# mit-han-lab/qserve

Measured on NVIDIA H100. Metric: tokens/s Llama-3-8B W4A8KV4 decode b64, higher is better.
Workload: dtype s8

## Files before the change

### qserve_b200/csrc/gemm.cu

```cuda
#include <cstdarg>
#include <cstdio>
#include <cstdlib>
#include <cstring>
#include <mutex>
#include <unordered_map>

#include "common.cuh"
#include "launch.h"

namespace qs {

namespace {

constexpr int kBM = 128;
constexpr int kBK = 128;
constexpr int kSub = 2;
constexpr int kConsumers = 128;
constexpr int kNumThreads = 192;
constexpr int kFrag = 4;

enum { kModeW4Chn = 0, kModeW4Grp = 1, kModeW8 = 2 };

struct GemmParams {
  const uint8_t* s2_scales;
  const uint8_t* s2_zeros;
  const __half* wscales;
  const __half* w_szs;
  const __half* ascales;
  const __half* a_ssums;
  __half* out;
  int32_t* acc_out;
  int M, N, K;
  int m_tiles, kb_per_tile, split;
  unsigned long long* prof;
};

template <int MODE, int NT, int WS, int AS>
struct Cfg {
  static constexpr int kActSub = NT * kBK;
  static constexpr int kWSub = (MODE == kModeW8) ? kBM * kBK : kBM * kBK / 2;
  static constexpr int kS2Sub = (MODE == kModeW4Grp) ? 2 * kBM : 0;
  static constexpr int kActBytes = kSub * kActSub;
  static constexpr int kWBytes = kSub * kWSub;
  static constexpr int kS2Bytes = kSub * kS2Sub;
  static constexpr int kWStageTx = kWBytes + kS2Bytes;
  static constexpr int kOffAct = 0;
  static constexpr int kOffW = kOffAct + AS * kActBytes;
  static constexpr int kOffS2 = kOffW + WS * kWBytes;
  static constexpr int kPipeBytes = kOffS2 + WS * kS2Bytes;
  static constexpr int kRedBytes = NT * kBM * 4;
  static constexpr int kOffRow = (kPipeBytes > kRedBytes ? kPipeBytes : kRedBytes);
  static constexpr int kOffBar = kOffRow + 2 * NT * 4;
  static constexpr int kNumBars = 2 * WS + 2 * AS;
  static constexpr int kSmemBytes = kOffBar + kNumBars * 8;
  static constexpr int kCtasPerSm = (NT <= 64 && kSmemBytes <= 113 * 1024) ? 2 : 1;
  static_assert(kSmemBytes <= 227 * 1024, "shared memory overflow");
};

__device__ __forceinline__ unsigned long long gtime() {
  unsigned long long t;
  asm volatile("mov.u64 %0, %globaltimer;" : "=l"(t)::"memory");
  return t;
}
#define QS_PROF(slot) do { if (p.prof) p.prof[blockIdx.x * 16 + (slot)] = gtime(); } while (0)

__device__ __forceinline__ uint32_t cluster_ctarank() {
  uint32_t r;
  asm volatile("mov.u32 %0, %%cluster_ctarank;" : "=r"(r));
  return r;
}
__device__ __forceinline__ void cluster_sync_all() {
  asm volatile("barrier.cluster.arrive.release.aligned;\n\tbarrier.cluster.wait.acquire.aligned;" ::: "memory");
}
__device__ __forceinline__ void cluster_arrive() { asm volatile("barrier.cluster.arrive.release;" ::: "memory"); }
__device__ __forceinline__ void cluster_wait() { asm volatile("barrier.cluster.wait.acquire;" ::: "memory"); }
__device__ __forceinline__ uint32_t smid() {
  uint32_t r;
  asm volatile("mov.u32 %0, %%smid;" : "=r"(r));
  return r;
}
__device__ __forceinline__ uint32_t map_to_cta(uint32_t smem_addr, uint32_t rank) {
  uint32_t r;
  asm volatile("mapa.shared::cluster.u32 %0, %1, %2;" : "=r"(r) : "r"(smem_addr), "r"(rank));
  return r;
}
__device__ __forceinline__ void st_dsmem_u32(uint32_t addr, uint32_t v) {
  asm volatile("st.shared::cluster.u32 [%0], %1;" ::"r"(addr), "r"(v) : "memory");
}

template <int V>
struct IntTag { static constexpr int value = V; };

template <int MODE>
__device__ __forceinline__ float epilogue_one(int32_t acc, float ws, float wsz, float as, float asum) {
  float ps = __int2float_rn(acc);
  if constexpr (MODE == kModeW4Chn) {
    float t = __fmul_rn(__fmul_rn(ps, ws), as);
    float u = __fmul_rn(wsz, asum);
    return __fsub_rn(t, u);
  } else {
    return __fmul_rn(ps, __fmul_rn(ws, as));
  }
}

template <int MODE>
__device__ __forceinline__ int acc_channel(int h, int w, int r) {
  return (MODE == kModeW8) ? 64 * h + 16 * w + r : 32 * w + 16 * h + r;
}

template <int MODE, int NT, int WS, int AS, bool ACC>
__global__ void __launch_bounds__(kNumThreads, Cfg<MODE, NT, WS, AS>::kCtasPerSm)
gemm_kernel(const __grid_constant__ CUtensorMap tmap_act, const __grid_constant__ CUtensorMap tmap_w, const GemmParams p) {
  using C = Cfg<MODE, NT, WS, AS>;
  extern __shared__ __align__(1024) uint8_t smem[];
  if (threadIdx.x == 0 && (smem_u32(smem) & 1023u) != 0) __trap();
  uint8_t* s_act = smem + C::kOffAct;
  uint8_t* s_w = smem + C::kOffW;
  uint8_t* s_s2 = smem + C::kOffS2;
  int32_t* s_red = reinterpret_cast<int32_t*>(smem);
  float* s_asc = reinterpret_cast<float*>(smem + C::kOffRow);
  float* s_asum = s_asc + NT;
  uint64_t* bar_wfull = reinterpret_cast<uint64_t*>(smem + C::kOffBar);
  uint64_t* bar_wempty = bar_wfull + WS;
  uint64_t* bar_xfull = bar_wempty + WS;
  uint64_t* bar_xempty = bar_xfull + AS;

  const int warp = threadIdx.x >> 5;
  const int lane = threadIdx.x & 31;
  const int S = p.split;
  const int rank = (S > 1) ? static_cast<int>(cluster_ctarank()) : 0;
  const int tile = blockIdx.x / S;
  const int m_tile = tile % p.m_tiles, n_tile = tile / p.m_tiles;
  const int KB = p.kb_per_tile;
  const int kb_begin = (KB * rank) / S, kb_end = (KB * (rank + 1)) / S;
  const int n_kb = kb_end - kb_begin;
  if (threadIdx.x == 0) {
    QS_PROF(0);
    if (p.prof) p.prof[blockIdx.x * 16 + 15] = smid();
  }
  qs_trace(QS_K_GEMM, 0);

  if (threadIdx.x == 0) {
    tma_prefetch_desc(&tmap_act);
    tma_prefetch_desc(&tmap_w);
    for (int i = 0; i < WS; ++i) {
      mbar_init(&bar_wfull[i], 1);
      mbar_init(&bar_wempty[i], 4);
    }
    for (int i = 0; i < AS; ++i) {
      mbar_init(&bar_xfull[i], 1);
      mbar_init(&bar_xempty[i], 4);
    }
    fence_barrier_init();
  }
  __syncthreads();
  if (threadIdx.x == 0) { pdl_launch_dependents(); QS_PROF(1); }

  if (warp == 4) {
    if (lane == 0) {
      const int w_row = (MODE == kModeW8) ? n_tile * kBM : n_tile * 4;
      const uint8_t* s2s = p.s2_scales + static_cast<size_t>(n_tile) * kBM;
      const uint8_t* s2z = p.s2_zeros + static_cast<size_t>(n_tile) * kBM;
      int s = 0;
      uint32_t ph = 0;
      for (int it = 0; it < n_kb; ++it) {
        if (it >= WS) mbar_wait_nocall(&bar_wempty[s], ph);
        mbar_expect_tx(&bar_wfull[s], C::kWStageTx);
#pragma unroll
        for (int u = 0; u < kSub; ++u) {
          const int kb = (kb_begin + it) * kSub + u;
          tma_load_2d(s_w + s * C::kWBytes + u * C::kWSub, &tmap_w, (MODE == kModeW8) ? kb * kBK : kb * 256, w_row, &bar_wfull[s]);
          if constexpr (MODE == kModeW4Grp) {
            const int kg = kb < p.K / kBK ? kb : p.K / kBK - 1;
            bulk_copy_g2s(s_s2 + s * C::kS2Bytes + u * C::kS2Sub, s2s + static_cast<size_t>(kg) * p.N, kBM, &bar_wfull[s]);
            bulk_copy_g2s(s_s2 + s * C::kS2Bytes + u * C::kS2Sub + kBM, s2z + static_cast<size_t>(kg) * p.N, kBM, &bar_wfull[s]);
          }
        }
        if (++s == WS) { s = 0; if (it >= WS) ph ^= 1; }
      }
      QS_PROF(3);
    }
  } else if (warp == 5) {
    if (lane == 0) {
      const int a_row = m_tile * NT;
      pdl_wait();
      QS_PROF(2);
      qs_trace(QS_K_GEMM, 1, 5 * 32);
      int s = 0;
      uint32_t ph = 0;
      for (int it = 0; it < n_kb; ++it) {
        if (it >= AS) mbar_wait_nocall(&bar_xempty[s], ph);
        mbar_expect_tx(&bar_xfull[s], C::kActBytes);
#pragma unroll
        for (int u = 0; u < kSub; ++u)
          tma_load_2d(s_act + s * C::kActBytes + u * C::kActSub, &tmap_act, ((kb_begin + it) * kSub + u) * kBK, a_row, &bar_xfull[s]);
        if (++s == AS) { s = 0; if (it >= AS) ph ^= 1; }
      }
    }
  } else {
    int32_t acc[2][NT / 2];
#pragma unroll
    for (int h = 0; h < 2; ++h)
#pragma unroll
      for (int i = 0; i < NT / 2; ++i) acc[h][i] = 0;
    mbar_wait_nocall(&bar_wfull[0], 0);
    mbar_wait_nocall(&bar_xfull[0], 0);
    if (threadIdx.x == 0) QS_PROF(4);
    const bool leader = lane == 0;
    int sw = 0, sx = 0, prev_sw = WS - 1, prev_sx = AS - 1;
    uint32_t phw = 0, phx = 0;
    for (int it = 0; it < n_kb; ++it) {
      mbar_wait_nocall(&bar_wfull[sw], phw);
      mbar_wait_nocall(&bar_xfull[sx], phx);
      if constexpr (MODE == kModeW8) {
#pragma unroll
        for (int u = 0; u < kSub; ++u) {
          const uint64_t bdesc = gmma_desc_sw128(smem_u32(s_act + sx * C::kActBytes + u * C::kActSub));
          const uint64_t adesc = gmma_desc_sw128(smem_u32(s_w + sw * C::kWBytes + u * C::kWSub));
          wgmma_fence();
#pragma unroll
          for (int t = 0; t < kBK / 32; ++t) {
            wgmma_s8_ss(acc[0], adesc + t * 2, bdesc + t * 2);
            wgmma_s8_ss(acc[1], adesc + (64 * kBK >> 4) + t * 2, bdesc + t * 2);
          }
          wgmma_commit();
        }
        wgmma_wait<kSub>();
        mbar_arrive_if(&bar_wempty[prev_sw], it > 0 && leader);
        mbar_arrive_if(&bar_xempty[prev_sx], it > 0 && leader);
      } else {
        uint32_t fr[kFrag][2][4];
#pragma unroll
        for (int u = 0; u < kSub; ++u) {
          const uint64_t bdesc = gmma_desc_sw128(smem_u32(s_act + sx * C::kActBytes + u * C::kActSub));
          const uint8_t* wsrc = s_w + sw * C::kWBytes + u * C::kWSub + warp * 2048 + lane * 16;
          uint32_t sc4 = 0, zp4 = 0;
          if constexpr (MODE == kModeW4Grp) {
            const uint8_t* s2 = s_s2 + sw * C::kS2Bytes + u * C::kS2Sub + warp * 32 + (lane >> 2) * 4;
            sc4 = *reinterpret_cast<const uint32_t*>(s2);
            zp4 = *reinterpret_cast<const uint32_t*>(s2 + kBM);
          }
#pragma unroll
          for (int t = 0; t < 4; ++t) {
            const int j = u * 4 + t;
            const uint4 v = *reinterpret_cast<const uint4*>(wsrc + t * 512);
            uint32_t xl = v.x & 0x0F0F0F0Fu, xh = (v.x >> 4) & 0x0F0F0F0Fu;
            uint32_t yl = v.y & 0x0F0F0F0Fu, yh = (v.y >> 4) & 0x0F0F0F0Fu;
            uint32_t zl = v.z & 0x0F0F0F0Fu, zh = (v.z >> 4) & 0x0F0F0F0Fu;
            uint32_t wl = v.w & 0x0F0F0F0Fu, wh = (v.w >> 4) & 0x0F0F0F0Fu;
            if constexpr (MODE == kModeW4Grp) {
              const uint32_t s0 = sc4 & 0xFF, s1 = (sc4 >> 8) & 0xFF, s2 = (sc4 >> 16) & 0xFF, s3 = sc4 >> 24;
              const uint32_t z0 = __byte_perm(zp4, 0, 0x0000), z1 = __byte_perm(zp4, 0, 0x1111);
              const uint32_t z2 = __byte_perm(zp4, 0, 0x2222), z3 = __byte_perm(zp4, 0, 0x3333);
              xl = __vadd4(xl * s0, z0); zl = __vadd4(zl * s0, z0);
              yl = __vadd4(yl * s1, z1); wl = __vadd4(wl * s1, z1);
              xh = __vadd4(xh * s2, z2); zh = __vadd4(zh * s2, z2);
              yh = __vadd4(yh * s3, z3); wh = __vadd4(wh * s3, z3);
            }
            wgmma_wait<kFrag - 1>();
            if (j == kFrag - 1) mbar_arrive_if(&bar_xempty[prev_sx], it > 0 && leader);
            uint32_t(&f)[2][4] = fr[j % kFrag];
            f[0][0] = xl; f[0][1] = yl; f[0][2] = zl; f[0][3] = wl;
            f[1][0] = xh; f[1][1] = yh; f[1][2] = zh; f[1][3] = wh;
            wgmma_fence();
            wgmma_s8_rs(acc[0], f[0], bdesc + t * 2);
            wgmma_s8_rs(acc[1], f[1], bdesc + t * 2);
            wgmma_commit();
          }
        }
        mbar_arrive_if(&bar_wempty[sw], leader);
      }
      prev_sw = sw;
      prev_sx = sx;
      if (++sw == WS) { sw = 0; phw ^= 1; }
      if (++sx == AS) { sx = 0; phx ^= 1; }
    }
    wgmma_wait<0>();
    if (threadIdx.x == 0) QS_PROF(6);
    if (S > 1) cluster_arrive();

    const int epi_tid = threadIdx.x;
    pdl_wait();
    const int m0 = m_tile * NT;
    for (int j = epi_tid; j < NT; j += kConsumers) {
      const bool ok = (m0 + j) < p.M;
      s_asc[j] = ok ? __half2float(p.ascales[m0 + j]) : 0.f;
      if constexpr (MODE == kModeW4Chn) s_asum[j] = ok ? __half2float(p.a_ssums[m0 + j]) : 0.f;
    }
    if (S > 1) cluster_wait(); else named_bar_sync(1, kConsumers);
    if (epi_tid == 0) QS_PROF(8);
    const int r0 = lane >> 2, c0 = (lane & 3) * 2;
    if (S == 1) {
#pragma unroll
      for (int h = 0; h < 2; ++h)
#pragma unroll
        for (int i = 0; i < NT / 2; ++i) {
          const int ch = acc_channel<MODE>(h, warp, r0 + 8 * ((i >> 1) & 1));
          const int tok = (i >> 2) * 8 + c0 + (i & 1);
          s_red[tok * kBM + ch] = acc[h][i];
        }
    } else {
      const int cps = kBM / S;
      const uint32_t rx_base = smem_u32(s_red);
#pragma unroll
      for (int h = 0; h < 2; ++h)
#pragma unroll
        for (int i = 0; i < NT / 2; ++i) {
          const int ch = acc_channel<MODE>(h, warp, r0 + 8 * ((i >> 1) & 1));
          const int tok = (i >> 2) * 8 + c0 + (i & 1);
          const uint32_t owner = static_cast<uint32_t>(ch / cps);
          st_dsmem_u32(map_to_cta(rx_base, owner) + static_cast<uint32_t>(((rank * NT + tok) * cps + ch % cps) * 4), static_cast<uint32_t>(acc[h][i]));
        }
    }
    if (epi_tid == 0) QS_PROF(9);
  }
  if (S > 1 && threadIdx.x >= kConsumers) { cluster_arrive(); cluster_wait(); }

  if (S > 1) cluster_sync_all(); else __syncthreads();
  if (threadIdx.x < kConsumers) {
    pdl_wait();
    const int tid = threadIdx.x;
    if (tid == 0) QS_PROF(10);
    const int npairs = 64 / S;
    const int pr = (64 * rank) / S + tid % npairs;
    const float ws0 = __half2float(__ldg(p.wscales + n_tile * kBM + 2 * pr)), ws1 = __half2float(__ldg(p.wscales + n_tile * kBM + 2 * pr + 1));
    float wz0 = 0.f, wz1 = 0.f;
    if constexpr (MODE == kModeW4Chn) {
      wz0 = __half2float(__ldg(p.w_szs + n_tile * kBM + 2 * pr));
      wz1 = __half2float(__ldg(p.w_szs + n_tile * kBM + 2 * pr + 1));
    }
    const int m0 = m_tile * NT;
    const int tstep = kConsumers / npairs;
    const int n = n_tile * kBM + 2 * pr;
    const int tok_end = min(NT, p.M - m0);
    const int tok0 = tid / npairs;
    const uint32_t off0 = static_cast<uint32_t>((tok0 * kBM + 2 * pr) * 4), off_step = static_cast<uint32_t>(tstep * kBM * 4);
    __half* optr = p.out + static_cast<size_t>(m0 + tok0) * p.N + n;
    const size_t ostep = static_cast<size_t>(tstep) * p.N;
    auto finish = [&](int tok, int2 acc, __half* dst) {
      const float as = s_asc[tok], asum = s_asum[tok];
      const float o0 = epilogue_one<MODE>(acc.x, ws0, wz0, as, asum);
      const float o1 = epilogue_one<MODE>(acc.y, ws1, wz1, as, asum);
      *reinterpret_cast<__half2*>(dst) = __floats2half2_rn(o0, o1);
      if constexpr (ACC) *reinterpret_cast<int2*>(p.acc_out + (dst - p.out)) = acc;
    };
    if (S == 1) {
      constexpr int kPerThread = NT / 2;
#pragma unroll 1
      for (int i0 = 0; i0 < kPerThread; i0 += 16) {
        int2 v[16];
#pragma unroll
        for (int e = 0; e < 16; ++e)
          if (kPerThread > e) v[e] = *reinterpret_cast<const int2*>(reinterpret_cast<const uint8_t*>(s_red) + off0 + (i0 + e) * off_step);
#pragma unroll
        for (int e = 0; e < 16; ++e) {
          const int tok = tok0 + (i0 + e) * tstep;
          if (kPerThread > e && tok < tok_end) finish(tok, v[e], optr + (i0 + e) * ostep);
        }
      }
    } else {
      const int cps = kBM / S;
      const int32_t* rx = s_red;
      const int prl = tid % npairs;
      auto reduce_rows = [&](auto s_tag) {
        constexpr int SS = decltype(s_tag)::value;
        constexpr int TPT = NT / (2 * SS) > 0 ? NT / (2 * SS) : 1;
        int2 v[TPT][SS];
#pragma unroll
        for (int i = 0; i < TPT; ++i) {
          const int tok = tok0 + i * tstep;
#pragma unroll
          for (int r = 0; r < SS; ++r)
            v[i][r] = (tok < NT) ? *reinterpret_cast<const int2*>(rx + (r * NT + tok) * cps + 2 * prl) : make_int2(0, 0);
        }
#pragma unroll
        for (int i = 0; i < TPT; ++i) {
          const int tok = tok0 + i * tstep;
          int2 acc = v[i][0];
#pragma unroll
          for (int r = 1; r < SS; ++r) { acc.x += v[i][r].x; acc.y += v[i][r].y; }
          if (tok < tok_end) finish(tok, acc, optr + i * ostep);
        }
      };
      if (S == 2) reduce_rows(IntTag<2>{});
      else if (S == 4) reduce_rows(IntTag<4>{});
      else reduce_rows(IntTag<8>{});
    }
    if (tid == 0) QS_PROF(11);
  } else {
    pdl_wait();
  }
  if (threadIdx.x == 0) QS_PROF(12);
  qs_trace(QS_K_GEMM, 2);
}


typedef CUresult (*PFN_encodeTiled)(CUtensorMap*, CUtensorMapDataType, cuuint32_t, void*, const cuuint64_t*, const cuuint64_t*,
                                    const cuuint32_t*, const cuuint32_t*, CUtensorMapInterleave, CUtensorMapSwizzle,
                                    CUtensorMapL2promotion, CUtensorMapFloatOOBfill);

PFN_encodeTiled get_encode() {
  static PFN_encodeTiled fn = nullptr;
  if (!fn) {
    void* p = nullptr;
    cudaDriverEntryPointQueryResult q;
    if (cudaGetDriverEntryPoint("cuTensorMapEncodeTiled", &p, cudaEnableDefault, &q) == cudaSuccess && p) fn = reinterpret_cast<PFN_encodeTiled>(p);
  }
  return fn;
}

struct TmapKey {
  const void* ptr; uint64_t a, b; uint32_t box, kind;
  bool operator==(const TmapKey& o) const { return ptr == o.ptr && a == o.a && b == o.b && box == o.box && kind == o.kind; }
};
struct TmapKeyHash {
  size_t operator()(const TmapKey& k) const {
    size_t h = reinterpret_cast<size_t>(k.ptr) * 0x9E3779B97F4A7C15ull;
    h ^= (k.a + 0x7F4A7C15ull + (h << 6) + (h >> 2));
    h ^= (k.b * 0xC2B2AE3D27D4EB4Full + (h << 6) + (h >> 2));
    return h ^ (static_cast<size_t>(k.box) << 7) ^ k.kind;
  }
};
std::unordered_map<TmapKey, CUtensorMap, TmapKeyHash>& tmap_cache() {
  static std::unordered_map<TmapKey, CUtensorMap, TmapKeyHash> c;
  return c;
}
std::mutex& tmap_mutex() { static std::mutex m; return m; }
bool tmap_lookup(const TmapKey& k, CUtensorMap* m) {
  std::lock_guard<std::mutex> g(tmap_mutex());
  auto it = tmap_cache().find(k);
  if (it == tmap_cache().end()) return false;
  memcpy(m, &it->second, sizeof(CUtensorMap));
  return true;
}
void tmap_store(const TmapKey& k, const CUtensorMap* m) {
  std::lock_guard<std::mutex> g(tmap_mutex());
  if (tmap_cache().size() > 16384) tmap_cache().clear();
  memcpy(&tmap_cache()[k], m, sizeof(CUtensorMap));
}

int make_tmap_u8(CUtensorMap* m, const void* ptr, uint64_t rows, uint64_t cols, uint32_t box_rows) {
  const TmapKey key{ptr, rows, cols, box_rows, 0u};
  if (tmap_lookup(key, m)) return QS_OK;
  PFN_encodeTiled enc = get_encode();
  if (!enc) return set_error(QS_ERR_CUDA, "cuTensorMapEncodeTiled entry point not available");
  cuuint64_t dims[2] = {cols, rows};
  cuuint64_t strides[1] = {cols};
  cuuint32_t box[2] = {128, box_rows};
  cuuint32_t estr[2] = {1, 1};
  CUresult r = enc(m, CU_TENSOR_MAP_DATA_TYPE_UINT8, 2, const_cast<void*>(ptr), dims, strides, box, estr, CU_TENSOR_MAP_INTERLEAVE_NONE,
                   CU_TENSOR_MAP_SWIZZLE_128B, CU_TENSOR_MAP_L2_PROMOTION_L2_256B, CU_TENSOR_MAP_FLOAT_OOB_FILL_NONE);
  if (r != CUDA_SUCCESS) return set_error(QS_ERR_CUDA, "cuTensorMapEncodeTiled failed (%d): ptr=%p rows=%llu cols=%llu box_rows=%u", (int)r, ptr,
                                          (unsigned long long)rows, (unsigned long long)cols, box_rows);
  tmap_store(key, m);
  return QS_OK;
}

int make_tmap_w4(CUtensorMap* m, const void* ptr, uint64_t N, uint64_t K, uint32_t box_bands = 4) {
  const TmapKey key{ptr, N, K, box_bands, 1u};
  if (tmap_lookup(key, m)) return QS_OK;
  PFN_encodeTiled enc = get_encode();
  if (!enc) return set_error(QS_ERR_CUDA, "cuTensorMapEncodeTiled entry point not available");
  cuuint64_t dims[2] = {K * 16 / 8, N / 32};
  cuuint64_t strides[1] = {K * 16};
  cuuint32_t box[2] = {256, box_bands};
  cuuint32_t estr[2] = {1, 1};
  CUresult r = enc(m, CU_TENSOR_MAP_DATA_TYPE_INT64, 2, const_cast<void*>(ptr), dims, strides, box, estr, CU_TENSOR_MAP_INTERLEAVE_NONE,
                   CU_TENSOR_MAP_SWIZZLE_NONE, CU_TENSOR_MAP_L2_PROMOTION_L2_256B, CU_TENSOR_MAP_FLOAT_OOB_FILL_NONE);
  if (r != CUDA_SUCCESS) return set_error(QS_ERR_CUDA, "cuTensorMapEncodeTiled(w4) failed (%d): ptr=%p N=%llu K=%llu", (int)r, ptr, (unsigned long long)N,
                                          (unsigned long long)K);
  tmap_store(key, m);
  return QS_OK;
}

int resident_clusters(const void* kern, int smem, int s) {
  int n = 0;
  if (s == 1) {
    if (cudaOccupancyMaxActiveBlocksPerMultiprocessor(&n, kern, kNumThreads, smem) != cudaSuccess) n = 0;
    return n * num_sms();
  }
  cudaLaunchConfig_t cfg{};
  cfg.gridDim = dim3(s);
  cfg.blockDim = dim3(kNumThreads);
  cfg.dynamicSmemBytes = smem;
  cudaLaunchAttribute attr;
  attr.id = cudaLaunchAttributeClusterDimension;
  attr.val.clusterDim.x = s;
  attr.val.clusterDim.y = 1;
  attr.val.clusterDim.z = 1;
  cfg.attrs = &attr;
  cfg.numAttrs = 1;
  if (cudaOccupancyMaxActiveClusters(&n, kern, &cfg) != cudaSuccess) n = 0;
  return n;
}

template <typename Resident>
int choose_split(int tiles, int kb_per_tile, int forced, Resident resident) {
  int s = 1;
  if (forced > 0) {
    s = forced;
  } else {
    while (s < 8 && kb_per_tile >= 4 * s && tiles <= resident(2 * s)) s *= 2;
  }
  while (s > 1 && kb_per_tile < s) s /= 2;
  return s;
}

template <int MODE, int NT, int WS, int AS>
int launch_gemm(const GemmArgs& a) {
  using C = Cfg<MODE, NT, WS, AS>;
  GemmParams p{};
  p.s2_scales = static_cast<const uint8_t*>(a.s2_scales);
  p.s2_zeros = static_cast<const uint8_t*>(a.s2_zeros);
  p.wscales = static_cast<const __half*>(a.wscales);
  p.w_szs = static_cast<const __half*>(a.w_szs);
  p.ascales = static_cast<const __half*>(a.ascales);
  p.a_ssums = static_cast<const __half*>(a.a_ssums);
  p.out = static_cast<__half*>(a.out);
  p.acc_out = static_cast<int32_t*>(a.acc_out);
  p.prof = static_cast<unsigned long long*>(a.prof);
  p.M = a.M; p.N = a.N; p.K = a.K;
  const int n_tiles = a.N / kBM;
  p.m_tiles = (a.M + NT - 1) / NT;
  p.kb_per_tile = (a.K + kSub * kBK - 1) / (kSub * kBK);
  const int tiles = n_tiles * p.m_tiles;

  CUtensorMap tm_act, tm_w;
  int rc = make_tmap_u8(&tm_act, a.act, a.M, a.K, NT);
  if (rc) return rc;
  rc = (MODE == kModeW8) ? make_tmap_u8(&tm_w, a.weight, a.N, a.K, kBM) : make_tmap_w4(&tm_w, a.weight, a.N, a.K);
  if (rc) return rc;

  auto kern = a.acc_out ? gemm_kernel<MODE, NT, WS, AS, true> : gemm_kernel<MODE, NT, WS, AS, false>;
  const int dev = device_ordinal();
  static bool attr_set[2][kMaxDevices] = {};
  bool& done = attr_set[a.acc_out ? 1 : 0][dev];
  if (!done) {
    rc = check_cuda(cudaFuncSetAttribute(kern, cudaFuncAttributeMaxDynamicSharedMemorySize, C::kSmemBytes), "cudaFuncSetAttribute(gemm smem)");
    if (rc) return rc;
    done = true;
  }
  static int resident_cache[2][kMaxDevices][4] = {};
  auto resident = [&](int s) {
    int& r = resident_cache[a.acc_out ? 1 : 0][dev][s == 1 ? 0 : s == 2 ? 1 : s == 4 ? 2 : 3];
    if (r == 0) r = resident_clusters(reinterpret_cast<const void*>(kern), C::kSmemBytes, s);
    return r;
  };
  p.split = choose_split(tiles, p.kb_per_tile, a.force_split, resident);
  if (p.prof)
    fprintf(stderr, "qs_gemm_plan mode=%d nt=%d ws=%d as=%d M=%d N=%d K=%d tiles=%d split=%d ctas=%d smem=%d resident_clusters=%d\n", MODE, NT, WS,
            AS, a.M, a.N, a.K, tiles, p.split, tiles * p.split, C::kSmemBytes, resident(p.split));
  cudaLaunchConfig_t cfg{};
  cfg.gridDim = dim3(tiles * p.split);
  cfg.blockDim = dim3(kNumThreads);
  cfg.dynamicSmemBytes = C::kSmemBytes;
  cfg.stream = static_cast<cudaStream_t>(a.stream);
  cudaLaunchAttribute attr[2];
  attr[0].id = cudaLaunchAttributeProgrammaticStreamSerialization;
  attr[0].val.programmaticStreamSerializationAllowed = pdl_enabled() ? 1 : 0;
  attr[1].id = cudaLaunchAttributeClusterDimension;
  attr[1].val.clusterDim.x = p.split;
  attr[1].val.clusterDim.y = 1;
  attr[1].val.clusterDim.z = 1;
  cfg.attrs = attr;
  cfg.numAttrs = 2;
  return check_cuda(cudaLaunchKernelEx(&cfg, kern, tm_act, tm_w, p), "gemm launch");
}

template <int MODE>
int dispatch_gemm(const GemmArgs& a) {
  QS_REQUIRE(a.M > 0 && a.N > 0 && a.K > 0, "gemm: empty problem M=%d N=%d K=%d", a.M, a.N, a.K);
  QS_REQUIRE(a.N % kBM == 0, "gemm: N=%d must be a multiple of %d", a.N, kBM);
  QS_REQUIRE(a.K % kBK == 0, "gemm: K=%d must be a multiple of %d", a.K, kBK);
  QS_REQUIRE((reinterpret_cast<uintptr_t>(a.act) & 15) == 0 && (reinterpret_cast<uintptr_t>(a.weight) & 15) == 0, "gemm: operands must be 16-byte aligned");
  QS_REQUIRE(a.force_split == 0 || a.force_split == 1 || a.force_split == 2 || a.force_split == 4 || a.force_split == 8, "gemm: split must be 1, 2, 4 or 8");
  constexpr bool w8 = (MODE == kModeW8), grp = (MODE == kModeW4Grp);
  QS_REQUIRE(a.force_nt == 0 || a.force_nt == 32 || a.force_nt == 64 || a.force_nt == 128, "gemm: tile tokens must be 32, 64 or 128");
  const int nt = a.force_nt > 0 ? a.force_nt : a.M <= 32 ? 32 : a.M <= 64 ? 64 : 128;
  if (nt == 32) return launch_gemm<MODE, 32, (w8 ? 2 : grp ? 4 : 5), 4>(a);
  if (nt == 64) return launch_gemm<MODE, 64, (w8 ? 2 : grp ? 3 : 4), (w8 ? 2 : 3)>(a);
  return launch_gemm<MODE, 128, 4, 2>(a);
}

}

int gemm_w4a8_per_chn(const GemmArgs& a) { return dispatch_gemm<kModeW4Chn>(a); }
int gemm_w4a8_per_group(const GemmArgs& a) { return dispatch_gemm<kModeW4Grp>(a); }
int gemm_w8a8(const GemmArgs& a) { return dispatch_gemm<kModeW8>(a); }
size_t gemm_workspace_bytes() { return 4096; }
int gemm_trace_install(void* buf, unsigned cap) { return qs_trace_install(buf, cap); }

}
```

Before: 14090.

## Use lane-contiguous DSMEM layout for split-K cluster reduction in GEMM epilogue

Changes the split-K cluster reduction buffer from a token-by-channel layout to one where each warp lane writes consecutive words, so remote DSMEM stores coalesce instead of scattering. The reduce phase is rewritten so warps walk rows of this layout, sum across ranks, and use a shuffle to pair adjacent channels before applying scales and writing half2 outputs. This aims to cut DSMEM store and shared-memory read bank conflicts during the epilogue. In exchange, scale loads move into the inner loop, where they are reloaded per row, and half the lanes sit idle on the store.

```diff
diff --git a/qserve_b200/csrc/gemm.cu b/qserve_b200/csrc/gemm.cu
--- a/qserve_b200/csrc/gemm.cu
+++ b/qserve_b200/csrc/gemm.cu
@@ -301,15 +301,18 @@
         }
     } else {
       const int cps = kBM / S;
+      constexpr int Q = NT / 4;
+      const int G = cps / 8;
       const uint32_t rx_base = smem_u32(s_red);
 #pragma unroll
       for (int h = 0; h < 2; ++h)
 #pragma unroll
-        for (int i = 0; i < NT / 2; ++i) {
-          const int ch = acc_channel<MODE>(h, warp, r0 + 8 * ((i >> 1) & 1));
-          const int tok = (i >> 2) * 8 + c0 + (i & 1);
-          const uint32_t owner = static_cast<uint32_t>(ch / cps);
-          st_dsmem_u32(map_to_cta(rx_base, owner) + static_cast<uint32_t>(((rank * NT + tok) * cps + ch % cps) * 4), static_cast<uint32_t>(acc[h][i]));
+        for (int hi = 0; hi < 2; ++hi) {
+          const int ch0 = acc_channel<MODE>(h, warp, 8 * hi);
+          const uint32_t dst = map_to_cta(rx_base, static_cast<uint32_t>(ch0 / cps)) +
+                               static_cast<uint32_t>(((rank * G + (ch0 % cps) / 8) * Q * 32 + lane) * 4);
+#pragma unroll
+          for (int q = 0; q < Q; ++q) st_dsmem_u32(dst + q * 128, static_cast<uint32_t>(acc[h][(q >> 1) * 4 + hi * 2 + (q & 1)]));
         }
     }
     if (epi_tid == 0) QS_PROF(9);
@@ -360,26 +363,47 @@
       }
     } else {
       const int cps = kBM / S;
-      const int32_t* rx = s_red;
-      const int prl = tid % npairs;
+      constexpr int Q = NT / 4;
+      const int G = cps / 8;
+      const int32_t* rx = s_red + lane;
+      const int nrows = G * Q;
+      const bool pair_lead = ((lane >> 2) & 1) == 0;
       auto reduce_rows = [&](auto s_tag) {
         constexpr int SS = decltype(s_tag)::value;
-        constexpr int TPT = NT / (2 * SS) > 0 ? NT / (2 * SS) : 1;
-        int2 v[TPT][SS];
-#pragma unroll
-        for (int i = 0; i < TPT; ++i) {
-          const int tok = tok0 + i * tstep;
-#pragma unroll
-          for (int r = 0; r < SS; ++r)
-            v[i][r] = (tok < NT) ? *reinterpret_cast<const int2*>(rx + (r * NT + tok) * cps + 2 * prl) : make_int2(0, 0);
-        }
-#pragma unroll
-        for (int i = 0; i < TPT; ++i) {
-          const int tok = tok0 + i * tstep;
-          int2 acc = v[i][0];
-#pragma unroll
-          for (int r = 1; r < SS; ++r) { acc.x += v[i][r].x; acc.y += v[i][r].y; }
-          if (tok < tok_end) finish(tok, acc, optr + i * ostep);
+        constexpr int kChunk = 4;
+#pragma unroll 1
+        for (int row0 = warp; row0 < nrows; row0 += 4 * kChunk) {
+          int32_t v[kChunk][SS];
+#pragma unroll
+          for (int c = 0; c < kChunk; ++c)
+#pragma unroll
+            for (int r = 0; r < SS; ++r) {
+              const int row = row0 + 4 * c;
+              v[c][r] = row < nrows ? rx[((r * G) * Q + row) * 32] : 0;
+            }
+#pragma unroll
+          for (int c = 0; c < kChunk; ++c) {
+            const int row = row0 + 4 * c;
+            int32_t sum = v[c][0];
+#pragma unroll
+            for (int r = 1; r < SS; ++r) sum += v[c][r];
+            const int32_t next = __shfl_down_sync(0xffffffffu, sum, 4);
+            const int j = row / Q, q = row % Q;
+            const int tok = (q >> 1) * 8 + (lane & 3) * 2 + (q & 1);
+            if (row < nrows && pair_lead && tok < tok_end) {
+              const int cn = n_tile * kBM + rank * cps + 8 * j + (lane >> 2);
+              const float cw0 = __half2float(__ldg(p.wscales + cn)), cw1 = __half2float(__ldg(p.wscales + cn + 1));
+              float cz0 = 0.f, cz1 = 0.f;
+              if constexpr (MODE == kModeW4Chn) {
+                cz0 = __half2float(__ldg(p.w_szs + cn));
+                cz1 = __half2float(__ldg(p.w_szs + cn + 1));
+              }
+              const float as = s_asc[tok], asum = s_asum[tok];
+              __half* dst = p.out + static_cast<size_t>(m0 + tok) * p.N + cn;
+              *reinterpret_cast<__half2*>(dst) = __floats2half2_rn(epilogue_one<MODE>(sum, cw0, cz0, as, asum), epilogue_one<MODE>(next, cw1, cz1, as, asum));
+              if constexpr (ACC) *reinterpret_cast<int2*>(p.acc_out + (dst - p.out)) = make_int2(sum, next);
+            }
+          }
         }
       };
       if (S == 2) reduce_rows(IntTag<2>{});
```

Result: no change. 14220, median of 6 (+0.9%).
